# spool-labs/clay

Hardware: AMD Instinct MI355X
Metric: device-resident encode GiB/s at (k=10,m=4,d=13); % of HBM roofline (higher is better)
Workload: dtype u8; 1 GPU; (k=10,m=4,d=13) encode, one 1 GiB stripe per GPU; stripe_input_bytes=1073741824, padded_stripe_bytes=1073745920, chunk_bytes=107374592, sub_chunk_bytes=419432, alpha=256, parallelism=stripe-per-gpu x1

## Files before the change

bench_tools/stream_probe.hip:

```cpp
#include <hip/hip_runtime.h>

#include <algorithm>
#include <cstdlib>
#include <cstdio>
#include <vector>

#include "../clay_amd/csrc/stream_encode.hpp"

using namespace clay::bs;

template <int L, int PROBE>
static float run(BsArgs a, int reps) {
    using Kn = StreamEnc<10, L>;
    (void)hipFuncSetAttribute(reinterpret_cast<const void *>(&k_stream_encode<10, L, PROBE>),
                              hipFuncAttributeMaxDynamicSharedMemorySize, Kn::LDS_BYTES);
    hipEvent_t e0, e1;
    (void)hipEventCreate(&e0);
    (void)hipEventCreate(&e1);
    std::vector<float> t;
    for (int r = 0; r < reps; r++) {
        (void)hipEventRecord(e0);
        k_stream_encode<10, L, PROBE><<<dim3(a.nslots * 8), dim3(Kn::BLOCK), Kn::LDS_BYTES>>>(a);
        (void)hipEventRecord(e1);
        (void)hipEventSynchronize(e1);
        float ms;
        (void)hipEventElapsedTime(&ms, e0, e1);
        if (r >= 3) t.push_back(ms);
    }
    std::sort(t.begin(), t.end());
    return t[t.size() / 2];
}

template <int L, int PROBE, int MAP = 0>
static float run_b2b(BsArgs a, int n, int warm = 50) {
    using Kn = StreamEnc<10, L>;
    (void)hipFuncSetAttribute(reinterpret_cast<const void *>(&k_stream_encode<10, L, PROBE, MAP>),
                              hipFuncAttributeMaxDynamicSharedMemorySize, Kn::LDS_BYTES);
    hipEvent_t e0, e1;
    (void)hipEventCreate(&e0);
    (void)hipEventCreate(&e1);
    for (int i = 0; i < warm; i++)
        k_stream_encode<10, L, PROBE, MAP><<<dim3(a.nslots * 8), dim3(Kn::BLOCK), Kn::LDS_BYTES>>>(a);
    (void)hipEventRecord(e0);
    for (int i = 0; i < n; i++)
        k_stream_encode<10, L, PROBE, MAP><<<dim3(a.nslots * 8), dim3(Kn::BLOCK), Kn::LDS_BYTES>>>(a);
    (void)hipEventRecord(e1);
    (void)hipEventSynchronize(e1);
    float ms;
    (void)hipEventElapsedTime(&ms, e0, e1);
    const hipError_t err = hipGetLastError();
    if (err != hipSuccess) {
        printf("HIP error (probe %d): %s\n", PROBE, hipGetErrorString(err));
        exit(3);
    }
    return ms / float(n);
}

template <int TP, int MAP = 0>
static void timing_report(BsArgs a, int n) {
    using Kn = StreamEnc<10, 4>;
    const int grid = int(a.nslots) * 8;
    const size_t rec = size_t(grid) * 12 * 24;
    uint64_t *tb;
    (void)hipMalloc(&tb, rec * 8);
    (void)hipMemset(tb, 0, rec * 8);
    a.par[4] = reinterpret_cast<uint8_t *>(tb);
    const float ms_plain = run_b2b<4, 0, MAP>(a, n);
    const float ms_tm = run_b2b<4, TP, MAP>(a, n);
    std::vector<uint64_t> h(rec);
    (void)hipMemcpy(h.data(), tb, rec * 8, hipMemcpyDeviceToHost);
    printf("b2b ms: plain %.4f  timing-probe %.4f (s_memtime counts per XCD; cycles below are per tile)\n", ms_plain, ms_tm);
    printf("wave  role     total   bar/vm y0   y1    y2 | math/bar y0   y1    y2 | issue y0  y1    y2 | end g0  g1    g2    g3\n");
    for (int w = 0; w < 12; w++) {
        double v[3][3] = {}, ge[4] = {}, tot = 0;
        int cnt = 0;
        for (int b = 0; b < grid; b++) {
            const uint64_t *p = &h[(size_t(b) * 12 + w) * 24];
            const double nt = double(p[16]);
// ... 19 lines not shown
    const bool quick = argc > 2;
    const size_t chunk = size_t(sc) * 256;
    uint8_t *data, *par;
    if (hipMalloc(&data, 10 * chunk) != hipSuccess || hipMalloc(&par, 4 * chunk) != hipSuccess) return 1;
    {
        std::vector<uint8_t> h(10 * chunk);
        uint64_t x = 0x9E3779B97F4A7C15ull;
        for (auto &b : h) { x ^= x << 13; x ^= x >> 7; x ^= x << 17; b = uint8_t(x >> 24); }
        (void)hipMemcpy(data, h.data(), h.size(), hipMemcpyHostToDevice);
    }
    BsArgs a{};
    for (int i = 0; i < 10; i++) a.data[i] = data + i * chunk;
    for (int x = 0; x < 4; x++) a.par[x] = par + x * chunk;
    a.sc = sc;
    const uint32_t ralign = argc > 3 ? uint32_t(atoi(argv[3])) : 32u;
    a.tiles_per_xcd = uint32_t(((sc + 7) / 8 + ralign - 1) / ralign * ralign);
    a.nslots = 32;
    const double bytes = 14.0 * chunk;
    auto rep = [&](const char *n, float ms) {
        printf("%-34s %8.4f ms  %7.1f GB/s (algorithmic)\n", n, ms, bytes / (ms * 1e-3) / 1e9);
        fflush(stdout);
    };
    (void)hipFuncSetAttribute(reinterpret_cast<const void *>(&k_stream_encode<10, 2, 0>),
                              hipFuncAttributeMaxDynamicSharedMemorySize, StreamEnc<10, 2>::LDS_BYTES);
    for (int i = 0; i < 300; i++) k_stream_encode<10, 2, 0><<<dim3(a.nslots * 8), dim3(StreamEnc<10, 2>::BLOCK), StreamEnc<10, 2>::LDS_BYTES>>>(a);
    {
        const hipError_t e = hipDeviceSynchronize();
        const hipError_t e2 = hipGetLastError();
        if (e != hipSuccess || e2 != hipSuccess) {
            printf("HIP error after warm-up: %s / %s\n", hipGetErrorString(e), hipGetErrorString(e2));
            return 3;
        }
    }
    if (argc > 2 && argv[2][0] == 't') {
        printf("sc %u segment timing\n", sc);
        timing_report<4096>(a, 200);
        printf("---- deferred end of group (PROBE 8192)\n");
        timing_report<4096 | 8192>(a, 200);
        return 0;
    }
    if (argc > 2 && argv[2][0] == 'd') {
        printf("sc %u deferred end-of-group A/B, back-to-back\n", sc);
        for (int rr = 0; rr < 3; rr++) {
            rep("b2b full", run_b2b<4, 0>(a, 200));
            rep("b2b full, end of group after the next barrier", run_b2b<4, 8192>(a, 200));
            rep("b2b memory only", run_b2b<4, 1>(a, 200));
            rep("b2b memory only, deferred", run_b2b<4, 8193>(a, 200));
            rep("b2b full, no sched barrier between nodes", run_b2b<4, 16384>(a, 200));
            rep("b2b full, sched barrier every 2 nodes", run_b2b<4, 32768>(a, 200));
            rep("b2b full, deferred + every 2 nodes", run_b2b<4, 32768 | 8192>(a, 200));
        }
        return 0;
    }
    if (argc > 2 && argv[2][0] == 'p') {
        printf("sc %u balanced priority A/B, back-to-back\n", sc);
        for (int rr = 0; rr < 3; rr++) {
            rep("b2b full", run_b2b<4, 0>(a, 200));
            rep("b2b full, balanced priority", run_b2b<4, 131072>(a, 200));
            rep("b2b math + stores (no DMA)", run_b2b<4, 2>(a, 200));
            rep("b2b math + stores (no DMA), balanced priority", run_b2b<4, 2 | 131072>(a, 200));
        }
        timing_report<4096 | 131072>(a, 200);
        return 0;
    }
    if (argc > 2 && argv[2][0] == 'v') {
        printf("sc %u variants, back-to-back (200 launches after 50 untimed)\n", sc);
// ... 201 lines not shown
            rep("L4 memory only, nt both", run<4, 321>(a, 15));
            rep("L4 reads, nt", run<4, 69>(a, 15));
            rep("L4 stores only, nt", run<4, 259>(a, 15));
        }
        return 0;
    }
    if (quick) {
        printf("sc %u\n", sc);
        for (int rr = 0; rr < 2; rr++) {
            rep("L4 full", run<4, 0>(a, 15));
            rep("L4 no math (memory only)", run<4, 1>(a, 15));
            rep("L4 reads", run<4, 5>(a, 15));
            rep("L4 stores only", run<4, 3>(a, 15));
            rep("L4 memory only, rotated stores", run<4, 33>(a, 15));
            rep("L4 stores only, rotated", run<4, 35>(a, 15));
        }
        return 0;
    }
    for (int rr = 0; rr < 2; rr++) {
        rep("L0 full", run<0, 0>(a, 15));
        rep("L1 full", run<1, 0>(a, 15));
        rep("L2 full", run<2, 0>(a, 15));
        rep("L4 full loaders prio 0", run<4, 8>(a, 15));
        rep("L4 full waves 4-7 prio 1", run<4, 16>(a, 15));
        rep("L2 full waves 4-7 prio 1", run<2, 16>(a, 15));
        rep("L4 full", run<4, 0>(a, 15));
        rep("L0 no math (memory only)", run<0, 1>(a, 15));
        rep("L4 no math (memory only)", run<4, 1>(a, 15));
        rep("L0 reads", run<0, 5>(a, 15));
        rep("L4 reads", run<4, 5>(a, 15));
        rep("L4 no DMA (math + stores)", run<4, 2>(a, 15));
        rep("L4 stores only", run<4, 3>(a, 15));
    }
    return 0;
}
```

clay_amd/csrc/engine.hip:

```cpp
#include <hip/hip_runtime.h>

#include <algorithm>
#include <atomic>
#include <cstdio>
#include <cstring>
#include <map>
#include <memory>
#include <mutex>
#include <set>
#include <string>
#include <thread>
#include <tuple>
#include <vector>

#include "../../include/clay.h"
#include "code.hpp"
#include "gf256.hpp"
#include "bitslice.hpp"
#include "stream_encode.hpp"
#include "repair_args.hpp"
#include "repair_batch_map.hpp"
#include "decode_args.hpp"
#include "line_args.hpp"
#include "kernels.hpp"
// ... 1148 lines not shown
    using Kn = bs::BsKernel<KD, M, PG>;
    using S = typename Kn::S;
    const clay_code_t &c = cs.code;
    if (int(c.k) != KD || int(c.m) != M || int(c.d) != KD + M - 1) return Error{};
    for (int p = 0; p < M; p++)
        for (int i = 0; i < S::K; i++)
            if (S::RS.g[p][i] != cs.rs.gen[(S::K + p) * S::K + i])
                return make_error(CLAY_ERR_DEVICE, 0, 0, 0, "bit-sliced RS table mismatch");
    const int per_cu = std::max(1, int((160 * 1024) / (Kn::LDS_WORDS * 4)));
    for (size_t s = 0; s < n_stripes; s++) {
        bs::BsArgs a{};
        for (int i = 0; i < S::K; i++) a.data[i] = i < KD ? data[s * KD + i] : nullptr;
        for (int x = 0; x < M; x++) a.par[x] = par[s * M + x];
        a.sc = sc;
        a.ntiles = uint32_t((sc + Kn::W - 1) / Kn::W);
        a.tiles_per_xcd = (a.ntiles + 7) / 8;
        const uint32_t max_slots = uint32_t(std::max(1, prop.multiProcessorCount / 8) * per_cu);
        a.nslots = std::min(max_slots, a.tiles_per_xcd);
        bool bt = sc % 8 != 0;
        for (int i = 0; i < KD; i++) bt |= (reinterpret_cast<uintptr_t>(a.data[i]) & 7u) != 0;
        for (int x = 0; x < M; x++) bt |= (reinterpret_cast<uintptr_t>(a.par[x]) & 7u) != 0;
        if (bt) bs::k_bs_encode<KD, M, PG, true><<<dim3(a.nslots * 8), dim3(Kn::BLOCK), 0, stream>>>(a);
        else bs::k_bs_encode<KD, M, PG><<<dim3(a.nslots * 8), dim3(Kn::BLOCK), 0, stream>>>(a);
        CLAY_HIP(hipGetLastError());
        t_last_launches++;
    }
    char buf[64];
    std::snprintf(buf, sizeof(buf), "bitsliced-k%dm%d-w%d", KD, M, Kn::W);
    t_last_path = buf;
    *done = true;
    return Error{};
}

template <int KD, int LOADERS>
static Error launch_stream(CodeState &cs, const DevProps &prop, const uint8_t *const *data, uint8_t *const *par,
                           size_t n_stripes, size_t sc, hipStream_t stream, bool *done) {
    using Kn = bs::StreamEnc<KD, LOADERS>;
    using S = typename Kn::S;
    const clay_code_t &c = cs.code;
    if (int(c.k) != KD || c.m != 4 || c.d != c.k + 3) return Error{};
    if (double(S::ALPHA) * double(sc) >= 4294967296.0 || sc < 16) return Error{};
    for (int p = 0; p < 4; p++)
        for (int i = 0; i < S::K; i++)
            if (S::RS.g[p][i] != cs.rs.gen[(S::K + p) * S::K + i])
                return make_error(CLAY_ERR_DEVICE, 0, 0, 0, "bit-sliced RS table mismatch");
    Error ae = lds_attr_once(reinterpret_cast<const void *>(&bs::k_stream_encode<KD, LOADERS, 0, bs::kStreamEncMap>),
                             Kn::LDS_BYTES, prop.dev);
    if (ae) return ae;
    const uint32_t region = uint32_t(((sc + 7) / 8 + 31) / 32 * 32);
    const uint32_t per_xcd = uint32_t(std::max(1, prop.cus / 8));
    const uint32_t nslots = std::min(per_xcd, std::max(1u, (region + 255u) / 256u));
    for (size_t s = 0; s < n_stripes; s++) {
        bs::BsArgs a{};
        for (int i = 0; i < S::K; i++) a.data[i] = i < KD ? data[s * KD + i] : nullptr;
        for (int x = 0; x < 4; x++) a.par[x] = par[s * 4 + x];
        a.sc = sc;
        a.tiles_per_xcd = region;
        a.nslots = nslots;
        a.ntiles = 0;
        bs::k_stream_encode<KD, LOADERS, 0, bs::kStreamEncMap><<<dim3(nslots * 8), dim3(Kn::BLOCK), Kn::LDS_BYTES, stream>>>(a);
        CLAY_HIP(hipGetLastError());
        t_last_launches++;
    }
    char buf[64];
    std::snprintf(buf, sizeof(buf), "stream-k%dm4-w256-l%d", KD, LOADERS);
    t_last_path = buf;
    *done = true;
    return Error{};
}

hipError_t launch_stream_encode3_kernel(int loaders, const bs::Enc3Args &a, hipStream_t stream, int dev);

static Error launch_stream3(CodeState &cs, const DevProps &prop, const uint8_t *const *data, uint8_t *const *par,
                            size_t n_stripes, size_t sc, hipStream_t stream, int loaders, bool *done) {
    using S = bs::Shape<9, 3>;
    const clay_code_t &c = cs.code;
    if (c.k != 9 || c.m != 3 || c.d != 11 || sc < 16 || double(S::ALPHA) * double(sc) >= 4294967296.0) return Error{};
    for (int p = 0; p < 3; p++)
        for (int i = 0; i < S::K; i++)
            if (S::RS.g[p][i] != cs.rs.gen[(S::K + p) * S::K + i])
                return make_error(CLAY_ERR_DEVICE, 0, 0, 0, "bit-sliced RS table mismatch");
    const uint32_t W = 512;
    bs::Enc3Args a{};
    a.sc = sc;
    a.region = uint32_t(((sc + 7) / 8 + 31) / 32 * 32);
    a.ns = std::min(uint32_t(std::max(1, prop.cus / 8)), std::max(1u, (a.region + W - 1) / W));
    for (size_t s = 0; s < n_stripes; s++) {
        for (int i = 0; i < 9; i++) a.data[i] = data[s * 9 + i];
        for (int x = 0; x < 3; x++) a.par[x] = par[s * 3 + x];
        CLAY_HIP(launch_stream_encode3_kernel(loaders, a, stream, prop.dev));
        t_last_launches++;
    }
    char buf[64];
    std::snprintf(buf, sizeof(buf), "stream3-k9m3-w512-l%d", loaders == 7 ? 7 : 2);
    t_last_path = buf;
    *done = true;
    return Error{};
}
// ... 26 lines not shown
        a.nslots = std::min(a.tiles_per_xcd, uint32_t(std::max(1, prop.cus / 8) * 8));
        CLAY_HIP(launch_bs_encode1_kernel(int(c.k), int(c.m), bt, a, stream));
        t_last_launches++;
    }
    char buf[64];
    std::snprintf(buf, sizeof(buf), "bitsliced-line-k%zum%zu-w%d", c.k, c.m, W);
    t_last_path = buf;
    *done = true;
    return Error{};
}

static Error encode_bitsliced(CodeState &cs, int dev, const uint8_t *const *data, uint8_t *const *par,
                              size_t n_stripes, size_t chunk, hipStream_t stream, int mode, int tile, bool *done) {
    *done = false;
    const clay_code_t &c = cs.code;
    const size_t sc = chunk / c.sub_chunk_no;
    if (c.d != c.k + c.m - 1) return Error{};
    bool rows8 = sc % 8 == 0;
    for (size_t s = 0; s < n_stripes && rows8; s++) {
        for (size_t i = 0; i < c.k; i++)
            if (reinterpret_cast<uintptr_t>(data[s * c.k + i]) % 8) rows8 = false;
        for (size_t i = 0; i < c.m; i++)
            if (reinterpret_cast<uintptr_t>(par[s * c.m + i]) % 8) rows8 = false;
    }
    const DevProps &prop = dev_props(dev);
    Error e;
    const int key = int(c.k * 100 + c.m);
    if (key == 903 && (mode == kModeStream || mode == kModeAuto)) {
        e = launch_stream3(cs, prop, data, par, n_stripes, sc, stream, tile == 7 ? 7 : 2, done);
        if (e || *done || mode == kModeStream) return e;
    }
    if (rows8 && (mode == kModeStream || mode == kModeAuto)) {
        if (key == 1004 || key == 904) {
            const int l = tile ? tile : 4;
            if (key == 1004)
                e = l == 1 ? launch_stream<10, 1>(cs, prop, data, par, n_stripes, sc, stream, done)
                  : l == 4 ? launch_stream<10, 4>(cs, prop, data, par, n_stripes, sc, stream, done)
                           : launch_stream<10, 2>(cs, prop, data, par, n_stripes, sc, stream, done);
            else
                e = launch_stream<9, 4>(cs, prop, data, par, n_stripes, sc, stream, done);
        }
        if (e || *done || mode == kModeStream) return e;
    }
    if (key == 402 && (mode == kModeStream || mode == kModeAuto)) {
        e = launch_bs_encode1(cs, prop, data, par, n_stripes, sc, stream, done);
        if (e || *done) return e;
    }
    if (mode == kModeStream) return e;
    switch (key) {
    case 1004:
        if (tile == 1) e = launch_bs<10, 4, 1>(cs, prop.raw, data, par, n_stripes, sc, stream, done);
        else if (tile == 4) e = launch_bs<10, 4, 4>(cs, prop.raw, data, par, n_stripes, sc, stream, done);
        else e = launch_bs<10, 4, 2>(cs, prop.raw, data, par, n_stripes, sc, stream, done);
        break;
    case 402: e = launch_bs<4, 2, 64>(cs, prop.raw, data, par, n_stripes, sc, stream, done); break;
    case 804: e = launch_bs<8, 4, 8>(cs, prop.raw, data, par, n_stripes, sc, stream, done); break;
    case 903: e = launch_bs<9, 3, 6>(cs, prop.raw, data, par, n_stripes, sc, stream, done); break;
    case 603: e = launch_bs<6, 3, 16>(cs, prop.raw, data, par, n_stripes, sc, stream, done); break;
    default: break;
    }
    return e;
}

static Error encode_staged(CodeState &cs, DevState &ds, int dev, const uint8_t *const *data, uint8_t *const *par,
                           size_t n_stripes, size_t chunk, hipStream_t stream) {
    const clay_code_t &c = cs.code;
    if (c.q * c.t > size_t(kMaxTn))
        return make_error(CLAY_ERR_DEVICE, c.q * c.t, 0, 0, "device engine supports at most %d internal nodes", kMaxTn);
    const Plan *pl = nullptr;
    Error pe = encode_plan(cs, &pl);
    if (pe) return pe;
// ... 1229 lines not shown
            if (outs[j].p)
                CLAY_HIP(hipMemcpy2DAsync(outs[j].p + off, sc, dout[j], wp, wp, outs[j].rows, hipMemcpyDeviceToHost, st));
    }
    for (int s = 0; s < ns; s++) CLAY_HIP(hipStreamSynchronize(r.st[s]));
    if (launches_out) *launches_out = launches;
    return Error{};
}

static int current_device(Error *e) {
    int ndev = 0, d = 0;
    if (hipGetDeviceCount(&ndev) != hipSuccess || ndev <= 0) {
        *e = make_error(CLAY_ERR_DEVICE, 0, 0, 0, "HIP error: no GPU device available (no CPU fallback)");
        return -1;
    }
    (void)hipGetDevice(&d);
    return d;
}

}

using namespace clay;

extern "C" {

int clay_abi_version(void) { return CLAY_ABI_VERSION; }
const char *clay_build_info(void) { return "clay_amd " __DATE__ " gfx950 HIP"; }
int clay_set_encode_path(int mode) {
    const int path = mode & 0xFF, tile = (mode >> 8) & 0xFF;
    if (mode < 0 || (mode >> 16) != 0) return -1;
    bool ok = false;
    switch (path) {
    case kModeAuto: case kModeStaged: case kModeFused: ok = tile == 0; break;
    case kModeBs: ok = tile == 0 || tile == 1 || tile == 4; break;
    case kModeStream: ok = tile == 0 || tile == 1 || tile == 2 || tile == 4 || tile == 7; break;
    default: ok = false;
    }
    if (!ok) return -1;
    const int prev = g_encode_mode.load() | (g_encode_tile.load() << 8);
    g_encode_tile.store(tile);
    g_encode_mode.store(path);
    return prev;
}
int clay_set_exec_mode(int mode) {
    if (mode != kExecAuto && mode != kExecGrouped && mode != kExecTile && mode != kExecStream &&
        mode != kExecStreamLocal && mode != kExecStreamFused2)
        return -1;
    return g_exec_mode.exchange(mode);
}
const char *clay_last_encode_path(void) { return t_last_path.c_str(); }
const char *clay_last_exec_path(void) { return t_last_exec; }
size_t clay_last_launch_count(void) { return t_last_launches; }

int clay_new(size_t k, size_t m, size_t d, clay_code_t *out, clay_error_t *err) {
    if (!out) return report(make_error(CLAY_ERR_INVALID_PARAMETERS, 0, 0, 0, "Invalid parameters: null output"), err);
    Error e = code_new(k, m, d, out);
    if (err) std::memset(err, 0, sizeof(*err));
    return e ? report(e, err) : 0;
}
int clay_new_default(size_t k, size_t m, clay_code_t *out, clay_error_t *err) {
    return clay_new(k, m, k + m - 1, out, err);
}
double clay_normalized_repair_bandwidth(const clay_code_t *c) {
    return double(c->d) / (double(c->k) * double(c->d - c->k + 1));
}
size_t clay_encoded_chunk_size(const clay_code_t *c, size_t len) { return encoded_chunk_size(*c, len); }

int clay_minimum_to_repair(const clay_code_t *code, size_t lost, const size_t *avail, size_t nav, size_t *helpers_out,
// ... 450 lines not shown
```

clay_amd/csrc/stream_encode.hpp:

```cpp
#pragma once

#include "encode_math.hpp"
#include "stream_tile_map.hpp"

namespace clay {
namespace bs {

__device__ __forceinline__ const uint8_t *uniform_ptr(const uint8_t *p) {
    const uint64_t v = reinterpret_cast<uint64_t>(p);
    const uint32_t lo = __builtin_amdgcn_readfirstlane(uint32_t(v)), hi = __builtin_amdgcn_readfirstlane(uint32_t(v >> 32));
    return reinterpret_cast<const uint8_t *>((uint64_t(hi) << 32) | lo);
}

__device__ __forceinline__ void dma16_masked(uint32_t lds_addr, const uint8_t *sbase, uint32_t voff, uint64_t mask) {
    unsigned keep;
    uint64_t ex;
    asm volatile(
        "s_mov_b32 %0, m0\n\ts_mov_b32 m0, %2\n\ts_mov_b64 %1, exec\n\ts_mov_b64 exec, %5\n\t"
        "global_load_lds_dwordx4 %3, %4\n\ts_mov_b64 exec, %1\n\ts_mov_b32 m0, %0"
        : "=&s"(keep), "=&s"(ex)
        : "s"(lds_addr), "v"(voff), "s"(sbase), "s"(mask)
        : "memory");
}

// ... 9 lines not shown
        nfull = len / round;
        const uint32_t left = len - nfull * round;
        const uint32_t wp = ((left + ns - 1) / ns + 31u) & ~31u;
        const uint32_t q0 = x0 + nfull * round + slot * wp;
        if (left && q0 < x1) {
            p0 = q0;
            p1 = q0 + wp < x1 ? q0 + wp : x1;
        }
    }
    __device__ int ntile() const { return int(nfull) + (p0 < p1 ? 1 : 0); }
    __device__ StreamTile tile(int k, uint32_t slot, uint32_t ns) const {
        if (uint32_t(k) < nfull) {
            const uint32_t b0 = x0 + (uint32_t(k) * ns + slot) * w;
            return {b0, b0 + w};
        }
        return {p0, p1};
    }
};

struct ChipMap {
    uint32_t b, G, nfull, pend, sc;
    __device__ ChipMap(uint32_t sc_, uint32_t b_, uint32_t G_) : b(b_), G(G_), nfull(sc_ / 256u), sc(sc_) {
        pend = (sc_ % 256u) && (nfull % G_) == b_ ? 1u : 0u;
    }
    __device__ int ntile() const { return int((nfull > b ? (nfull - b + G - 1) / G : 0u) + pend); }
    __device__ StreamTile tile(int k, uint32_t, uint32_t) const {
        const uint32_t t = b + uint32_t(k) * G;
        if (t < nfull) return {t * 256u, t * 256u + 256u};
        return {nfull * 256u, sc};
    }
};

template <int KD, int LOADERS, int CPL = 0, int CPS = 0, bool CSE = true, bool SINK = false, bool CHECK = false,
          int MAP = 0, bool LPRED = false>
struct StreamEnc {
    using K6 = EncMath<KD>;
    using S = typename K6::S;
    static constexpr int Q = 4, T = 4, W = 256, CWAVES = 8;
    static constexpr int BLOCK = 64 * (CWAVES + LOADERS);
    static constexpr int NODE_BYTES = 64 * W;
    static constexpr int REGION = Q * NODE_BYTES;
    static constexpr int LDS_BYTES = KD * NODE_BYTES;
    static constexpr int STEPS = 12;
    static constexpr int DMA_WAVES = LOADERS ? LOADERS : CWAVES;
    static constexpr int BPL = 16 / DMA_WAVES;
    static_assert(LOADERS == 0 || LOADERS == 1 || LOADERS == 2 || LOADERS == 4, "loader waves");
    static_assert(KD >= 9 && KD <= 10 && LDS_BYTES <= 160 * 1024, "one 16 KiB buffer per data node");

    static constexpr int nreal(int y) {
        int n = 0;
        for (int x = 0; x < Q; x++) n += (y * Q + x < KD);
        return n;
    }
    static constexpr int ninstr(int y) { return nreal(y) * BPL; }
    static constexpr int nstores(int g) { return 2 * (1 + 2 * g); }
    static constexpr int dshift(int y) { return 2 * (T - 2 - y); }

    __host__ __device__ static constexpr uint32_t sw(uint32_t r) { return ((r >> 1) & 1u) * 8u; }
    struct MapSpec {
        int kb0, kb1, kb2, wb, swb;
        bool light_old, pswap, redskip;
    };
    static constexpr MapSpec spec() {
        switch (MAP) {
            case 1: return {2, 3, 4, 5, 3, false, false, true};
            case 2: return {2, 3, 4, 5, 3, true, false, true};
            case 3: return {2, 3, 4, 5, 3, false, true, true};
            case 4: return {3, 2, 4, 5, 3, false, false, true};
            case 5: return {4, 3, 2, 5, 3, false, false, true};
            case 6: return {5, 4, 3, 2, 5, false, false, true};
            case 7: return {2, 5, 4, 3, 5, false, false, true};
            case 8: return {4, 5, 3, 2, 5, false, false, true};
            case 9: return {4, 5, 3, 2, 5, false, false, false};
            default: return {0, 1, 2, 3, 1, false, false, false};
        }
    }
    static constexpr MapSpec MS = spec();
    static constexpr bool PSWAP = MS.pswap;
    static constexpr uint32_t PAIR = MAP == 0 ? 4u : (4u << (PSWAP ? MS.kb1 : MS.kb0));
    __device__ static int colmap(int w, int k) {
        if constexpr (MAP == 0) return 8 * w + k;
        const int hi = MS.light_old ? (((w >> 2) & 1) ^ 1) : ((w >> 2) & 1);
        return (w & 1) | (hi << 1) | ((k & 1) << MS.kb0) | (((k >> 1) & 1) << MS.kb1) | (((k >> 2) & 1) << MS.kb2) |
               (((w >> 1) & 1) << MS.wb);
    }
    __host__ __device__ static constexpr uint32_t swn(uint32_t x, uint32_t r) {
        return MAP == 0 ? sw(r) : ((((r >> MS.swb) & 1u) ^ ((x >> 1) & 1u))) * 8u;
    }
    static constexpr bool sw_in_digit(int y) { return MS.swb == dshift(y) || MS.swb == dshift(y) + 1; }
    static constexpr int comp_swap(int y, int x) { return sw_in_digit(y) ? ((x >> (MS.swb - dshift(y))) & 1) : 0; }

    struct Loader {
        uint32_t off[2][BPL];
        uint32_t rl;
        uint32_t slot;
        int li;
    };
    __device__ static uint32_t k16_of(const Loader &L, int j, uint32_t b) {
        const uint32_t r = uint32_t(L.li * BPL + j) * 4u + L.rl;
        return (L.slot ^ swn(b * 2u, r)) * 16u;
    }
    __device__ static void loader_init(Loader &L, uint32_t sc, int li, int lane) {
        L.li = li;
        L.rl = uint32_t(lane) >> 4;
        L.slot = uint32_t(lane) & 15u;
#pragma unroll
        for (int j = 0; j < BPL; j++) {
            const uint32_t r = uint32_t(li * BPL + j) * 4u + L.rl;
            L.off[0][j] = r * 4u * sc + k16_of(L, j, 0u);
            L.off[1][j] = r * 4u * sc + k16_of(L, j, 1u);
        }
    }
    template <int Y>
    __device__ static void issue(const BsArgs &a, const Loader &L, uint32_t lds0, StreamTile t, int g) {
        const uint32_t sc = uint32_t(a.sc);
        const bool full = t.vend >= t.b0 + uint32_t(W);
        sfor<Q>([&](auto xc) BS_INL {
            constexpr int x = decltype(xc)::value;
            constexpr int node = Y * Q + x;
            if constexpr (node < KD) {
                constexpr uint32_t b = (uint32_t(x) >> 1) & 1u;
                const uint32_t dst = lds0 + uint32_t(node * NODE_BYTES) + uint32_t(L.li * BPL) * 1024u;
                if (full) {
                    const uint8_t *base = uniform_ptr(a.data[node] + (uint64_t(g) * sc + t.b0));
#pragma unroll
                    for (int j = 0; j < BPL; j++) dma16p<CPL>(dst + uint32_t(j) * 1024u, base, L.off[b][j]);
                } else if (LPRED && ((t.vend - t.b0) & 15u) == 0) {
                    const uint8_t *base = uniform_ptr(a.data[node] + (uint64_t(g) * sc + t.b0));
#pragma unroll
                    for (int j = 0; j < BPL; j++) {
                        const uint64_t mask = __builtin_amdgcn_ballot_w64(k16_of(L, j, b) + 16u <= t.vend - t.b0);
                        dma16_masked(dst + uint32_t(j) * 1024u, base, L.off[b][j], mask);
                    }
                } else {
                    const uint8_t *base = uniform_ptr(a.data[node] + uint64_t(g) * sc);
#pragma unroll
                    for (int j = 0; j < BPL; j++) {
                        const uint32_t k16 = k16_of(L, j, b);
                        uint32_t pos = t.b0 + k16;
                        if (pos + 16u > t.vend) pos = t.vend - 16u;
                        dma16p<CPL>(dst + uint32_t(j) * 1024u, base, L.off[b][j] - k16 + pos);
                    }
                }
            }
        });
    }
    __device__ static void issue_any(int y, const BsArgs &a, const Loader &L, uint32_t lds0, StreamTile t, int g) {
        if (y == 0) issue<0>(a, L, lds0, t, g);
        else if (y == 1) issue<1>(a, L, lds0, t, g);
        else issue<2>(a, L, lds0, t, g);
    }
    template <int Y>
    __device__ static void patch(const BsArgs &a, const Loader &L, uint8_t *smem, StreamTile t, int g, int lane) {
        const uint32_t sc = uint32_t(a.sc);
        sfor<Q>([&](auto xc) BS_INL {
            constexpr int x = decltype(xc)::value;
            constexpr int node = Y * Q + x;
            if constexpr (node < KD) {
#pragma unroll
                for (int j = 0; j < BPL; j++) {
                    const uint32_t pos = t.b0 + k16_of(L, j, (uint32_t(x) >> 1) & 1u);
                    if (!(pos < t.vend && pos + 16u > t.vend)) continue;
                    const int blk = L.li * BPL + j;
                    const uint32_t layer = (uint32_t(blk) * 4u + L.rl) * 4u + uint32_t(g);
                    const uint2 gv = *reinterpret_cast<const uint2 *>(a.data[node] + uint64_t(layer) * sc + pos);
                    *reinterpret_cast<uint4 *>(smem + node * NODE_BYTES + blk * 1024 + lane * 16) =
                        make_uint4(gv.x, gv.y, 0u, 0u);
                }
            }
        });
    }
    __device__ static void patch_any(int y, const BsArgs &a, const Loader &L, uint8_t *smem, StreamTile t, int g,
                                     int lane) {
        if (y == 0) patch<0>(a, L, smem, t, g, lane);
        else if (y == 1) patch<1>(a, L, smem, t, g, lane);
        else patch<2>(a, L, smem, t, g, lane);
    }

    struct LaneS {
        uint32_t own[2], cb[3][2];
        int cy[3];
    };
    __device__ static LaneS lane_consts(int c, int part) {
        LaneS L;
        if constexpr (MAP != 0) {
            const uint32_t uc = uint32_t(c), up = uint32_t(part);
            L.own[0] = uc * 256u + ((up ^ (((uc >> MS.swb) & 1u) * 8u)) * 16u);
// ... 195 lines not shown
                if (uint64_t(off) + 16u > lim || uint64_t(off) + PAIR * a.sc + 16u > lim) {
                    atomicOr(reinterpret_cast<unsigned int *>(a.par[5]), 1u << X);
                    return;
                }
            }
            st16sp<CPS>(base, off, lo[0], lo[1], lo[2], lo[3]);
            st16sp<CPS>(base, off + PAIR * uint32_t(a.sc), hi[0], hi[1], hi[2], hi[3]);
        } else {
            uint8_t *p = a.par[X] + uint64_t(z) * a.sc + t.b0 + prel;
#pragma unroll
            for (int h = 0; h < 2; h++) {
                const uint32_t pos = t.b0 + prel + 128u * uint32_t(h);
                const uint32_t nv = pos >= t.vend ? 0u : (t.vend - pos >= 16u ? 16u : t.vend - pos);
                if constexpr (CHECK) {
                    if (nv && (z >= 256u || pos + nv > a.sc)) {
                        atomicOr(reinterpret_cast<unsigned int *>(a.par[5]), 16u << X);
                        continue;
                    }
                }
                if (nv == 16u)
                    *reinterpret_cast<uint4 *>(p + 128 * h) = make_uint4(cv[4 * h], cv[4 * h + 1], cv[4 * h + 2], cv[4 * h + 3]);
                else if (nv >= 8u)
                    *reinterpret_cast<uint2 *>(p + 128 * h) = make_uint2(cv[4 * h], cv[4 * h + 1]);
            }
        }
    }
    template <int G>
    __device__ __forceinline__ static void end_group(const BsArgs &a, const uint32_t (&acc)[Q * 8], typename K6::Hold &H, int c,
                                     StreamTile t, uint32_t prel, bool ragged, uint32_t &sink) {
        const uint32_t zg = uint32_t(c * 4 + G);
        uint32_t cv[8];
#pragma unroll
        for (int w = 0; w < 8; w++) cv[w] = acc[G * 8 + w];
        put<G>(a, cv, zg, t, prel, ragged, sink);
        auto pair = [&](const uint32_t *uh_at_g, const uint32_t *ug_at_h, auto hc) BS_INL {
            constexpr int h = decltype(hc)::value;
            const uint32_t zh = uint32_t(c * 4 + h);
            uint32_t c12[16];
            if constexpr (CSE) {
                K6::pft_pair(uh_at_g, ug_at_h, c12);
            } else {
                uint32_t c1[8], c2[8];
                K6::pft(uh_at_g, ug_at_h, c1);
                K6::pft(ug_at_h, uh_at_g, c2);
#pragma unroll
                for (int w = 0; w < 8; w++) {
                    c12[w] = c1[w];
                    c12[8 + w] = c2[w];
                }
            }
            uint32_t c1[8], c2[8];
#pragma unroll
            for (int w = 0; w < 8; w++) {
                c1[w] = c12[w];
                c2[w] = c12[8 + w];
            }
            put<h>(a, c1, zg, t, prel, ragged, sink);
            put<G>(a, c2, zh, t, prel, ragged, sink);
        };
        auto keep = [&](int ri, int p) BS_INL {
#pragma unroll
            for (int w = 0; w < 8; w++) H.r[ri][w] = acc[p * 8 + w];
        };
        if constexpr (G == 0) {
            keep(0, 1);
            keep(1, 2);
            keep(2, 3);
        } else if constexpr (G == 1) {
            pair(acc + 0, H.r[0], std::integral_constant<int, 0>{});
            keep(0, 2);
            keep(3, 3);
        } else if constexpr (G == 2) {
            pair(acc + 0, H.r[1], std::integral_constant<int, 0>{});
            pair(acc + 8, H.r[0], std::integral_constant<int, 1>{});
            keep(1, 3);
        } else {
            pair(acc + 0, H.r[2], std::integral_constant<int, 0>{});
            pair(acc + 8, H.r[3], std::integral_constant<int, 1>{});
            pair(acc + 16, H.r[1], std::integral_constant<int, 2>{});
        }
    }
};

struct TimeAcc {
    uint64_t v[3][3] = {{0, 0, 0}, {0, 0, 0}, {0, 0, 0}}, gend[4] = {0, 0, 0, 0};
    uint64_t t_start = 0, t_first = 0, t_end = 0;
    __device__ __forceinline__ void add(int kind, int y, uint64_t &t0) {
        const uint64_t t1 = __builtin_amdgcn_s_memtime();
        const uint64_t d = t1 - t0;
        t0 = t1;
        if (y == 0) v[kind][0] += d;
        else if (y == 1) v[kind][1] += d;
        else v[kind][2] += d;
    }
    __device__ __forceinline__ void addg(int g, uint64_t &t0) {
        const uint64_t t1 = __builtin_amdgcn_s_memtime();
        const uint64_t d = t1 - t0;
        t0 = t1;
        if (g == 0) gend[0] += d;
        else if (g == 1) gend[1] += d;
        else if (g == 2) gend[2] += d;
        else gend[3] += d;
    }
    __device__ void put(uint64_t *p, int ntile) const {
        for (int i = 0; i < 3; i++)
            for (int j = 0; j < 3; j++) p[i * 3 + j] = v[i][j];
        for (int g = 0; g < 4; g++) p[9 + g] = gend[g];
        p[13] = t_start;
        p[14] = t_first;
        p[15] = t_end;
        p[16] = uint64_t(ntile);
    }
};

constexpr int kStreamEncMap = 8;

template <int KD, int LOADERS, int PROBE = 0, int MAP = 0>
__global__ __launch_bounds__((StreamEnc<KD, LOADERS>::BLOCK)) void k_stream_encode(BsArgs a) {
    using Kn = StreamEnc<KD, LOADERS, (PROBE >> 6) & 3, (PROBE >> 8) & 3, ((PROBE >> 10) & 1) == 0, (PROBE & 262144) != 0,
                         (PROBE & 524288) != 0, MAP, (PROBE & 4194304) != 0>;
    uint32_t sink = 0;
    constexpr bool TM = (PROBE & 4096) != 0;
    using K6 = typename Kn::K6;
    extern __shared__ __attribute__((aligned(16))) uint8_t smem[];
    const int wave = __builtin_amdgcn_readfirstlane(threadIdx.x >> 6), lane = threadIdx.x & 63;
    const uint32_t xcd = blockIdx.x & 7u, slot = blockIdx.x >> 3, ns = a.nslots;
    constexpr bool OLDMAP = (PROBE & (2048 | 2097152)) != 0;
    const auto tm = [&] {
        if constexpr ((PROBE & 2048) != 0) return ChipMap(uint32_t(a.sc), blockIdx.x, gridDim.x);
        else if constexpr (OLDMAP) return StreamMap(uint32_t(a.sc), a.tiles_per_xcd, ns, xcd, slot);
        else return BalancedMap(uint32_t(a.sc), a.tiles_per_xcd, ns, xcd, slot);
    }();
    const auto is_ragged = [](StreamTile t) BS_INL {
        return OLDMAP ? t.vend < t.b0 + uint32_t(Kn::W) : ((t.vend - t.b0) & 15u) != 0;
    };
    const int ntile = tm.ntile();
    if (ntile == 0) return;
    const int nsteps = ntile * Kn::STEPS;
    if (LOADERS > 0 && wave >= Kn::CWAVES) {
        if constexpr (!(PROBE & 8)) __builtin_amdgcn_s_setprio(3);
        typename Kn::Loader L;
        Kn::loader_init(L, uint32_t(a.sc), wave - Kn::CWAVES, lane);
        const uint32_t lds0 = lds_addr_of(smem);
        TimeAcc T;
        T.t_start = TM ? __builtin_amdgcn_s_memtime() : 0;
        if constexpr (!(PROBE & 2))
            for (int s = 0; s < 3 && s < nsteps; s++) Kn::issue_any(s % 3, a, L, lds0, tm.tile(0, slot, ns), s / 3);
        uint64_t t0 = TM ? __builtin_amdgcn_s_memtime() : 0;
        if constexpr (TM) T.t_first = t0;
        for (int s = 0; s < nsteps; s++) {
            const int k = s / Kn::STEPS, r = s % Kn::STEPS, g = r / 3, y = r % 3;
            const StreamTile t = tm.tile(k, slot, ns);
            int after = 0;
            if (s == 0) {
                after = (nsteps > 1 ? Kn::ninstr(1) : 0) + (nsteps > 2 ? Kn::ninstr(2) : 0);
            } else if (s + 1 < nsteps) {
                after = Kn::ninstr((y + 1) % 3);
            }
            const bool straddle = t.vend < t.b0 + uint32_t(Kn::W) && ((t.vend - t.b0) & 15u);
            if (PROBE & 2) {
            } else if (straddle) {
                wait_vm_n<0>();
                Kn::patch_any(y, a, L, smem, t, g, lane);
// ... 158 lines not shown
```

clay_amd/csrc/stream_tile_map.hpp:

```cpp
#pragma once

#include <cstdint>

#if defined(__HIPCC__) || defined(__CUDACC__)
#define CLAY_TILE_MAP_HD __host__ __device__
#else
#define CLAY_TILE_MAP_HD
#endif

namespace clay {
namespace bs {

struct StreamTile {
    uint32_t b0, vend;
};

struct BalancedMap {
    uint32_t x0, x1, nrounds, q, rem, nt;
    CLAY_TILE_MAP_HD BalancedMap(uint32_t sc, uint32_t region, uint32_t ns, uint32_t xcd, uint32_t slot) {
        x0 = xcd * region;
        x1 = x0 + region < sc ? x0 + region : sc;
        nrounds = q = rem = nt = 0;
        if (x0 >= x1) return;
        const uint32_t len = x1 - x0;
        nrounds = (len + ns * 256u - 1u) / (ns * 256u);
        const uint32_t pieces = (len + ns * 16u - 1u) / (ns * 16u);
        q = pieces / nrounds;
        rem = pieces % nrounds;
        nt = start(nrounds - 1u, slot, ns) < x1 ? nrounds : nrounds - 1u;
    }
    CLAY_TILE_MAP_HD uint32_t width(uint32_t r) const { return (q + (r < rem ? 1u : 0u)) * 16u; }
    CLAY_TILE_MAP_HD uint32_t start(uint32_t r, uint32_t slot, uint32_t ns) const {
        const uint32_t before = r * q + (r < rem ? r : rem);
        return x0 + (ns * before + slot * (q + (r < rem ? 1u : 0u))) * 16u;
    }
    CLAY_TILE_MAP_HD int rounds() const { return int(nrounds); }
    CLAY_TILE_MAP_HD int ntile() const { return int(nt); }
    CLAY_TILE_MAP_HD StreamTile tile(int k, uint32_t slot, uint32_t ns) const {
        const uint32_t b0 = start(uint32_t(k), slot, ns), e = b0 + width(uint32_t(k));
        return {b0, e < x1 ? e : x1};
    }
};

}
}
```

Measured before the change: 3301 GiB/s.

## Switch default stream encode to block-outermost load order and chip-interleaved tile map

Adds selectable read orders, store orders and a chip-wide interleaved tile map to the stream encode kernel. The production default becomes stream_ord(2,0,1): loads are issued block-by-block across all nodes, and tiles are spread over the whole chip instead of being confined to per-XCD regions. The goal is better HBM access locality and channel spread during the memory-bound encode. It also adds a probe sweep with byte-equality checks and a tile=16 escape hatch for the old order, at the cost of extra template instantiations.

```diff
diff --git a/bench_tools/stream_probe.hip b/bench_tools/stream_probe.hip
--- a/bench_tools/stream_probe.hip
+++ b/bench_tools/stream_probe.hip
@@ -31,19 +31,19 @@
     return t[t.size() / 2];
 }
 
-template <int L, int PROBE, int MAP = 0>
+template <int L, int PROBE, int MAP = 0, int ORD = 0>
 static float run_b2b(BsArgs a, int n, int warm = 50) {
     using Kn = StreamEnc<10, L>;
-    (void)hipFuncSetAttribute(reinterpret_cast<const void *>(&k_stream_encode<10, L, PROBE, MAP>),
+    (void)hipFuncSetAttribute(reinterpret_cast<const void *>(&k_stream_encode<10, L, PROBE, MAP, ORD>),
                               hipFuncAttributeMaxDynamicSharedMemorySize, Kn::LDS_BYTES);
     hipEvent_t e0, e1;
     (void)hipEventCreate(&e0);
     (void)hipEventCreate(&e1);
     for (int i = 0; i < warm; i++)
-        k_stream_encode<10, L, PROBE, MAP><<<dim3(a.nslots * 8), dim3(Kn::BLOCK), Kn::LDS_BYTES>>>(a);
+        k_stream_encode<10, L, PROBE, MAP, ORD><<<dim3(a.nslots * 8), dim3(Kn::BLOCK), Kn::LDS_BYTES>>>(a);
     (void)hipEventRecord(e0);
     for (int i = 0; i < n; i++)
-        k_stream_encode<10, L, PROBE, MAP><<<dim3(a.nslots * 8), dim3(Kn::BLOCK), Kn::LDS_BYTES>>>(a);
+        k_stream_encode<10, L, PROBE, MAP, ORD><<<dim3(a.nslots * 8), dim3(Kn::BLOCK), Kn::LDS_BYTES>>>(a);
     (void)hipEventRecord(e1);
     (void)hipEventSynchronize(e1);
     float ms;
@@ -129,6 +129,72 @@
             return 3;
         }
     }
+    if (argc > 2 && argv[2][0] == 'o') {
+        constexpr int M = kStreamEncMap;
+        printf("sc %u order sweep, back-to-back (200 launches after 50 untimed)\n", sc);
+        const size_t pbytes = 4 * chunk;
+        std::vector<uint8_t> ref(pbytes), got(pbytes);
+        (void)hipMemset(par, 0, pbytes);
+        run_b2b<4, 0, M, 0>(a, 1, 0);
+        (void)hipDeviceSynchronize();
+        (void)hipMemcpy(ref.data(), par, pbytes, hipMemcpyDeviceToHost);
+        bool all_equal = true;
+        auto check = [&](const char *name, float) {
+            (void)hipDeviceSynchronize();
+            (void)hipMemcpy(got.data(), par, pbytes, hipMemcpyDeviceToHost);
+            printf("  %-10s bytes == R0/S0: %s\n", name, ref == got ? "yes" : "NO");
+            all_equal = all_equal && ref == got;
+            (void)hipMemset(par, 0xA5, pbytes);
+        };
+        (void)hipMemset(par, 0xA5, pbytes);
+#ifndef STREAM_PROBE_COMBO_A
+#define STREAM_PROBE_COMBO_A stream_ord(2, 0, 1)
+#endif
+#ifndef STREAM_PROBE_COMBO_B
+#define STREAM_PROBE_COMBO_B stream_ord(2, 2, 1)
+#endif
+        constexpr int CA = STREAM_PROBE_COMBO_A, CB = STREAM_PROBE_COMBO_B;
+        if (argv[2][1] == 'c') {
+            printf("combination A: R%d S%d M%d, B: R%d S%d M%d\n", CA & 3, (CA >> 2) & 3, CA >> 4, CB & 3, (CB >> 2) & 3, CB >> 4);
+            check("A", run_b2b<4, 0, M, CA>(a, 1, 0));
+            check("B", run_b2b<4, 0, M, CB>(a, 1, 0));
+            if (!all_equal) return 4;
+            for (int rr = 0; rr < 3; rr++) {
+                rep("b2b full, R0 S0 M0", run_b2b<4, 0, M, 0>(a, 200));
+                rep("b2b full, combination A", run_b2b<4, 0, M, CA>(a, 200));
+                rep("b2b full, combination B", run_b2b<4, 0, M, CB>(a, 200));
+                rep("b2b memory only, R0 S0 M0", run_b2b<4, 1, M, 0>(a, 200));
+                rep("b2b memory only, combination A", run_b2b<4, 1, M, CA>(a, 200));
+                rep("b2b memory only, combination B", run_b2b<4, 1, M, CB>(a, 200));
+            }
+            return 0;
+        }
+        check("R1", run_b2b<4, 0, M, stream_ord(1, 0, 0)>(a, 1, 0));
+        check("R2", run_b2b<4, 0, M, stream_ord(2, 0, 0)>(a, 1, 0));
+        check("R3", run_b2b<4, 0, M, stream_ord(3, 0, 0)>(a, 1, 0));
+        check("S1", run_b2b<4, 0, M, stream_ord(0, 1, 0)>(a, 1, 0));
+        check("S2", run_b2b<4, 0, M, stream_ord(0, 2, 0)>(a, 1, 0));
+        check("M1", run_b2b<4, 0, M, stream_ord(0, 0, 1)>(a, 1, 0));
+        if (!all_equal) return 4;
+        for (int rr = 0; rr < 3; rr++) {
+            rep("b2b full, R0 S0 M0", run_b2b<4, 0, M, 0>(a, 200));
+            rep("b2b full, R1", run_b2b<4, 0, M, stream_ord(1, 0, 0)>(a, 200));
+            rep("b2b full, R2", run_b2b<4, 0, M, stream_ord(2, 0, 0)>(a, 200));
+            rep("b2b full, R3", run_b2b<4, 0, M, stream_ord(3, 0, 0)>(a, 200));
+            rep("b2b full, S1", run_b2b<4, 0, M, stream_ord(0, 1, 0)>(a, 200));
+            rep("b2b full, S2", run_b2b<4, 0, M, stream_ord(0, 2, 0)>(a, 200));
+            rep("b2b full, M1", run_b2b<4, 0, M, stream_ord(0, 0, 1)>(a, 200));
+            rep("b2b memory only, R0 S0 M0", run_b2b<4, 1, M, 0>(a, 200));
+            rep("b2b memory only, R1", run_b2b<4, 1, M, stream_ord(1, 0, 0)>(a, 200));
+            rep("b2b memory only, R2", run_b2b<4, 1, M, stream_ord(2, 0, 0)>(a, 200));
+            rep("b2b memory only, R3", run_b2b<4, 1, M, stream_ord(3, 0, 0)>(a, 200));
+            rep("b2b memory only, S1", run_b2b<4, 1, M, stream_ord(0, 1, 0)>(a, 200));
+            rep("b2b memory only, S2", run_b2b<4, 1, M, stream_ord(0, 2, 0)>(a, 200));
+            rep("b2b memory only, M1", run_b2b<4, 1, M, stream_ord(0, 0, 1)>(a, 200));
+        }
+        return 0;
+    }
+#ifndef STREAM_PROBE_ORDERS_ONLY
     if (argc > 2 && argv[2][0] == 't') {
         printf("sc %u segment timing\n", sc);
         timing_report<4096>(a, 200);
@@ -396,5 +462,6 @@
         rep("L4 no DMA (math + stores)", run<4, 2>(a, 15));
         rep("L4 stores only", run<4, 3>(a, 15));
     }
+#endif
     return 0;
 }
diff --git a/clay_amd/csrc/engine.hip b/clay_amd/csrc/engine.hip
--- a/clay_amd/csrc/engine.hip
+++ b/clay_amd/csrc/engine.hip
@@ -1204,7 +1204,7 @@
     return Error{};
 }
 
-template <int KD, int LOADERS>
+template <int KD, int LOADERS, int ORD = bs::kStreamEncOrd>
 static Error launch_stream(CodeState &cs, const DevProps &prop, const uint8_t *const *data, uint8_t *const *par,
                            size_t n_stripes, size_t sc, hipStream_t stream, bool *done) {
     using Kn = bs::StreamEnc<KD, LOADERS>;
@@ -1216,7 +1216,7 @@
         for (int i = 0; i < S::K; i++)
             if (S::RS.g[p][i] != cs.rs.gen[(S::K + p) * S::K + i])
                 return make_error(CLAY_ERR_DEVICE, 0, 0, 0, "bit-sliced RS table mismatch");
-    Error ae = lds_attr_once(reinterpret_cast<const void *>(&bs::k_stream_encode<KD, LOADERS, 0, bs::kStreamEncMap>),
+    Error ae = lds_attr_once(reinterpret_cast<const void *>(&bs::k_stream_encode<KD, LOADERS, 0, bs::kStreamEncMap, ORD>),
                              Kn::LDS_BYTES, prop.dev);
     if (ae) return ae;
     const uint32_t region = uint32_t(((sc + 7) / 8 + 31) / 32 * 32);
@@ -1230,12 +1230,12 @@
         a.tiles_per_xcd = region;
         a.nslots = nslots;
         a.ntiles = 0;
-        bs::k_stream_encode<KD, LOADERS, 0, bs::kStreamEncMap><<<dim3(nslots * 8), dim3(Kn::BLOCK), Kn::LDS_BYTES, stream>>>(a);
+        bs::k_stream_encode<KD, LOADERS, 0, bs::kStreamEncMap, ORD><<<dim3(nslots * 8), dim3(Kn::BLOCK), Kn::LDS_BYTES, stream>>>(a);
         CLAY_HIP(hipGetLastError());
         t_last_launches++;
     }
     char buf[64];
-    std::snprintf(buf, sizeof(buf), "stream-k%dm4-w256-l%d", KD, LOADERS);
+    std::snprintf(buf, sizeof(buf), "stream-k%dm4-w256-l%d-r%ds%dm%d", KD, LOADERS, ORD & 3, (ORD >> 2) & 3, ORD >> 4);
     t_last_path = buf;
     *done = true;
     return Error{};
@@ -1328,11 +1328,14 @@
     }
     if (rows8 && (mode == kModeStream || mode == kModeAuto)) {
         if (key == 1004 || key == 904) {
-            const int l = tile ? tile : 4;
-            if (key == 1004)
-                e = l == 1 ? launch_stream<10, 1>(cs, prop, data, par, n_stripes, sc, stream, done)
+            const int l = tile == 16 ? 4 : tile ? tile : 4;
+            if (tile == 16)
+                e = key == 1004 ? launch_stream<10, 4, 0>(cs, prop, data, par, n_stripes, sc, stream, done)
+                                : launch_stream<9, 4, 0>(cs, prop, data, par, n_stripes, sc, stream, done);
+            else if (key == 1004)
+                e = l == 1 ? launch_stream<10, 1, 0>(cs, prop, data, par, n_stripes, sc, stream, done)
                   : l == 4 ? launch_stream<10, 4>(cs, prop, data, par, n_stripes, sc, stream, done)
-                           : launch_stream<10, 2>(cs, prop, data, par, n_stripes, sc, stream, done);
+                           : launch_stream<10, 2, 0>(cs, prop, data, par, n_stripes, sc, stream, done);
             else
                 e = launch_stream<9, 4>(cs, prop, data, par, n_stripes, sc, stream, done);
         }
@@ -2628,7 +2631,7 @@
     switch (path) {
     case kModeAuto: case kModeStaged: case kModeFused: ok = tile == 0; break;
     case kModeBs: ok = tile == 0 || tile == 1 || tile == 4; break;
-    case kModeStream: ok = tile == 0 || tile == 1 || tile == 2 || tile == 4 || tile == 7; break;
+    case kModeStream: ok = tile == 0 || tile == 1 || tile == 2 || tile == 4 || tile == 7 || tile == 16; break;
     default: ok = false;
     }
     if (!ok) return -1;
diff --git a/clay_amd/csrc/stream_encode.hpp b/clay_amd/csrc/stream_encode.hpp
--- a/clay_amd/csrc/stream_encode.hpp
+++ b/clay_amd/csrc/stream_encode.hpp
@@ -65,7 +65,7 @@
 };
 
 template <int KD, int LOADERS, int CPL = 0, int CPS = 0, bool CSE = true, bool SINK = false, bool CHECK = false,
-          int MAP = 0, bool LPRED = false>
+          int MAP = 0, bool LPRED = false, int RORD = 0, int SORD = 0>
 struct StreamEnc {
     using K6 = EncMath<KD>;
     using S = typename K6::S;
@@ -78,6 +78,9 @@
     static constexpr int DMA_WAVES = LOADERS ? LOADERS : CWAVES;
     static constexpr int BPL = 16 / DMA_WAVES;
     static_assert(LOADERS == 0 || LOADERS == 1 || LOADERS == 2 || LOADERS == 4, "loader waves");
+    static_assert(RORD >= 0 && RORD <= 3 && SORD >= 0 && SORD <= 2, "read / store order");
+    static_assert(!(LPRED && RORD == 1), "masked loads are not built for the node-major order");
+    static_assert(!(RORD == 2 && LOADERS == 1), "the block-outermost order is not built for one loader wave");
     static_assert(KD >= 9 && KD <= 10 && LDS_BYTES <= 160 * 1024, "one 16 KiB buffer per data node");
 
     static constexpr int nreal(int y) {
@@ -125,10 +128,28 @@
 
     struct Loader {
         uint32_t off[2][BPL];
+        uint32_t offe[2];
         uint32_t rl;
         uint32_t slot;
         int li;
     };
+    static constexpr int SWB = MS.swb;
+    __device__ static uint32_t e_of(uint32_t blk, uint32_t b) {
+        const uint32_t eb = MAP == 0 ? 0u : b;
+        if constexpr (SWB >= 2) return eb ^ ((blk >> (SWB - 2)) & 1u);
+        else return eb;
+    }
+    __device__ static uint32_t k16_e(const Loader &L, uint32_t e) {
+        uint32_t lb = 0;
+        if constexpr (SWB < 2) lb = (L.rl >> SWB) & 1u;
+        return (L.slot ^ ((e ^ lb) * 8u)) * 16u;
+    }
+    template <int Y>
+    __device__ static void item_r1(const Loader &L, int i, uint32_t &x, uint32_t &blk) {
+        const uint32_t entry = uint32_t(L.li * ninstr(Y) + i);
+        x = entry >> 4;
+        blk = entry & 15u;
+    }
     __device__ static uint32_t k16_of(const Loader &L, int j, uint32_t b) {
         const uint32_t r = uint32_t(L.li * BPL + j) * 4u + L.rl;
         return (L.slot ^ swn(b * 2u, r)) * 16u;
@@ -143,11 +164,63 @@
             L.off[0][j] = r * 4u * sc + k16_of(L, j, 0u);
             L.off[1][j] = r * 4u * sc + k16_of(L, j, 1u);
         }
+        if constexpr (RORD == 1) {
+            L.offe[0] = L.rl * 4u * sc + k16_e(L, 0u);
+            L.offe[1] = L.rl * 4u * sc + k16_e(L, 1u);
+        }
     }
     template <int Y>
     __device__ static void issue(const BsArgs &a, const Loader &L, uint32_t lds0, StreamTile t, int g) {
         const uint32_t sc = uint32_t(a.sc);
         const bool full = t.vend >= t.b0 + uint32_t(W);
+        if constexpr (RORD == 1) {
+#pragma unroll
+            for (int i = 0; i < ninstr(Y); i++) {
+                uint32_t x, blk;
+                item_r1<Y>(L, i, x, blk);
+                const uint32_t e = e_of(blk, (x >> 1) & 1u);
+                const uint32_t dst = lds0 + (uint32_t(Y * Q) + x) * uint32_t(NODE_BYTES) + blk * 1024u;
+                const uint8_t *row0 = a.data[Y * Q + x] + (uint64_t(blk) * 16u + uint64_t(g)) * sc;
+                if (full) {
+                    dma16p<CPL>(dst, uniform_ptr(row0 + t.b0), e ? L.offe[1] : L.offe[0]);
+                } else {
+                    const uint32_t k16 = k16_e(L, e);
+                    uint32_t pos = t.b0 + k16;
+                    if (pos + 16u > t.vend) pos = t.vend - 16u;
+                    dma16p<CPL>(dst, uniform_ptr(row0), L.rl * 4u * sc + pos);
+                }
+            }
+            return;
+        }
+        if constexpr (RORD == 2) {
+            const uint8_t *bases[Q];
+            sfor<Q>([&](auto xc) BS_INL {
+                constexpr int x = decltype(xc)::value;
+                if constexpr (Y * Q + x < KD)
+                    bases[x] = uniform_ptr(a.data[Y * Q + x] + (uint64_t(g) * sc + (full ? t.b0 : 0u)));
+            });
+#pragma unroll
+            for (int j = 0; j < BPL; j++) {
+                sfor<Q>([&](auto xc) BS_INL {
+                    constexpr int x = decltype(xc)::value;
+                    constexpr int node = Y * Q + x;
+                    if constexpr (node < KD) {
+                        constexpr uint32_t b = (uint32_t(x) >> 1) & 1u;
+                        const uint32_t dst = lds0 + uint32_t(node * NODE_BYTES) + uint32_t(L.li * BPL + j) * 1024u;
+                        if (full) {
+                            dma16p<CPL>(dst, bases[x], L.off[b][j]);
+                        } else {
+                            const uint32_t k16 = k16_of(L, j, b);
+                            uint32_t pos = t.b0 + k16;
+                            if (pos + 16u > t.vend) pos = t.vend - 16u;
+                            dma16p<CPL>(dst, bases[x], L.off[b][j] - k16 + pos);
+                        }
+                    }
+                });
+            }
+            return;
+        }
+        constexpr auto blk_of = [](int j) { return RORD == 3 ? BPL - 1 - j : j; };
         sfor<Q>([&](auto xc) BS_INL {
             constexpr int x = decltype(xc)::value;
             constexpr int node = Y * Q + x;
@@ -157,7 +230,10 @@
                 if (full) {
                     const uint8_t *base = uniform_ptr(a.data[node] + (uint64_t(g) * sc + t.b0));
 #pragma unroll
-                    for (int j = 0; j < BPL; j++) dma16p<CPL>(dst + uint32_t(j) * 1024u, base, L.off[b][j]);
+                    for (int jj = 0; jj < BPL; jj++) {
+                        const int j = blk_of(jj);
+                        dma16p<CPL>(dst + uint32_t(j) * 1024u, base, L.off[b][j]);
+                    }
                 } else if (LPRED && ((t.vend - t.b0) & 15u) == 0) {
                     const uint8_t *base = uniform_ptr(a.data[node] + (uint64_t(g) * sc + t.b0));
 #pragma unroll
@@ -186,6 +262,21 @@
     template <int Y>
     __device__ static void patch(const BsArgs &a, const Loader &L, uint8_t *smem, StreamTile t, int g, int lane) {
         const uint32_t sc = uint32_t(a.sc);
+        if constexpr (RORD == 1) {
+#pragma unroll
+            for (int i = 0; i < ninstr(Y); i++) {
+                uint32_t x, blk;
+                item_r1<Y>(L, i, x, blk);
+                const uint32_t pos = t.b0 + k16_e(L, e_of(blk, (x >> 1) & 1u));
+                if (!(pos < t.vend && pos + 16u > t.vend)) continue;
+                const uint32_t node = uint32_t(Y * Q) + x;
+                const uint32_t layer = (blk * 4u + L.rl) * 4u + uint32_t(g);
+                const uint2 gv = *reinterpret_cast<const uint2 *>(a.data[node] + uint64_t(layer) * sc + pos);
+                *reinterpret_cast<uint4 *>(smem + node * uint32_t(NODE_BYTES) + blk * 1024u + uint32_t(lane) * 16u) =
+                    make_uint4(gv.x, gv.y, 0u, 0u);
+            }
+            return;
+        }
         sfor<Q>([&](auto xc) BS_INL {
             constexpr int x = decltype(xc)::value;
             constexpr int node = Y * Q + x;
@@ -447,7 +538,8 @@
         uint32_t cv[8];
 #pragma unroll
         for (int w = 0; w < 8; w++) cv[w] = acc[G * 8 + w];
-        put<G>(a, cv, zg, t, prel, ragged, sink);
+        if constexpr (SORD != 2) put<G>(a, cv, zg, t, prel, ragged, sink);
+        uint32_t held[G > 0 ? G : 1][8];
         auto pair = [&](const uint32_t *uh_at_g, const uint32_t *ug_at_h, auto hc) BS_INL {
             constexpr int h = decltype(hc)::value;
             const uint32_t zh = uint32_t(c * 4 + h);
@@ -470,8 +562,14 @@
                 c1[w] = c12[w];
                 c2[w] = c12[8 + w];
             }
-            put<h>(a, c1, zg, t, prel, ragged, sink);
-            put<G>(a, c2, zh, t, prel, ragged, sink);
+            if constexpr (SORD == 1) {
+                put<G>(a, c2, zh, t, prel, ragged, sink);
+#pragma unroll
+                for (int w = 0; w < 8; w++) held[h][w] = c1[w];
+            } else {
+                put<h>(a, c1, zg, t, prel, ragged, sink);
+                put<G>(a, c2, zh, t, prel, ragged, sink);
+            }
         };
         auto keep = [&](int ri, int p) BS_INL {
 #pragma unroll
@@ -494,6 +592,13 @@
             pair(acc + 8, H.r[3], std::integral_constant<int, 1>{});
             pair(acc + 16, H.r[1], std::integral_constant<int, 2>{});
         }
+        if constexpr (SORD == 1) {
+            sfor<G>([&](auto hc) BS_INL {
+                constexpr int h = decltype(hc)::value;
+                put<h>(a, held[h], zg, t, prel, ragged, sink);
+            });
+        }
+        if constexpr (SORD == 2) put<G>(a, cv, zg, t, prel, ragged, sink);
     }
 };
 
@@ -530,10 +635,14 @@
 
 constexpr int kStreamEncMap = 8;
 
-template <int KD, int LOADERS, int PROBE = 0, int MAP = 0>
+constexpr int stream_ord(int rord, int sord, int tmap) { return rord | (sord << 2) | (tmap << 4); }
+constexpr int kStreamEncOrd = stream_ord(2, 0, 1);
+
+template <int KD, int LOADERS, int PROBE = 0, int MAP = 0, int ORD = 0>
 __global__ __launch_bounds__((StreamEnc<KD, LOADERS>::BLOCK)) void k_stream_encode(BsArgs a) {
     using Kn = StreamEnc<KD, LOADERS, (PROBE >> 6) & 3, (PROBE >> 8) & 3, ((PROBE >> 10) & 1) == 0, (PROBE & 262144) != 0,
-                         (PROBE & 524288) != 0, MAP, (PROBE & 4194304) != 0>;
+                         (PROBE & 524288) != 0, MAP, (PROBE & 4194304) != 0, ORD & 3, (ORD >> 2) & 3>;
+    static_assert((ORD >> 5) == 0, "read order, store order, tile map");
     uint32_t sink = 0;
     constexpr bool TM = (PROBE & 4096) != 0;
     using K6 = typename Kn::K6;
@@ -544,6 +653,7 @@
     const auto tm = [&] {
         if constexpr ((PROBE & 2048) != 0) return ChipMap(uint32_t(a.sc), blockIdx.x, gridDim.x);
         else if constexpr (OLDMAP) return StreamMap(uint32_t(a.sc), a.tiles_per_xcd, ns, xcd, slot);
+        else if constexpr ((ORD & 16) != 0) return InterleavedMap(uint32_t(a.sc), a.tiles_per_xcd, ns, xcd, slot);
         else return BalancedMap(uint32_t(a.sc), a.tiles_per_xcd, ns, xcd, slot);
     }();
     const auto is_ragged = [](StreamTile t) BS_INL {
diff --git a/clay_amd/csrc/stream_tile_map.hpp b/clay_amd/csrc/stream_tile_map.hpp
--- a/clay_amd/csrc/stream_tile_map.hpp
+++ b/clay_amd/csrc/stream_tile_map.hpp
@@ -42,5 +42,16 @@
     }
 };
 
+struct InterleavedMap {
+    BalancedMap m;
+    uint32_t gslot, gns;
+    CLAY_TILE_MAP_HD InterleavedMap(uint32_t sc, uint32_t , uint32_t ns, uint32_t xcd, uint32_t slot)
+        : m(sc, sc, 8u * ns, 0u, xcd * ns + slot), gslot(xcd * ns + slot), gns(8u * ns) {}
+    CLAY_TILE_MAP_HD uint32_t width(uint32_t r) const { return m.width(r); }
+    CLAY_TILE_MAP_HD int rounds() const { return m.rounds(); }
+    CLAY_TILE_MAP_HD int ntile() const { return m.ntile(); }
+    CLAY_TILE_MAP_HD StreamTile tile(int k, uint32_t, uint32_t) const { return m.tile(k, gslot, gns); }
+};
+
 }
 }
```

New measurement: 3249 GiB/s. -1.6%, worse.
